# anenbergb/Co-DETR-TensorRT

Measured on AMD Instinct MI355X. Metric: images/sec, Co-DINO Swin-L 1920x1280 fp16 (p50 ms/image alongside), higher is better.
Workload: dtype f16

## Files before the change

co-detr-tensorrt_amd/csrc/gemm_xs.hip:

```cpp
#include "gemm_route.h"
#include "gemm_tile.h"

namespace {

#ifndef CODETR_XS_ABL
#define CODETR_XS_ABL 0
#endif
#ifdef CODETR_XS_STAMPS
__device__ unsigned long long* g_xs_stamps = nullptr;
#define XS_STAMP(i) xs_t[i] = __builtin_readcyclecounter()
#else
#define XS_STAMP(i)
#endif
struct XsPosGen {
  const float* ycum[5];
  const float* xcum[5];
  const unsigned short* level_embed;
  int H[5], W[5], start[5];
  int L, S;
  float log2_temperature, scale, eps, offset;
  int normalize;
};

template <class T, int KS, int ACT, bool HAS_RES, class OT = T, bool SPLIT = false, bool POSGEN = false>
__global__ __launch_bounds__(256) void linear_xs_kernel(const unsigned short* __restrict__ X,
                                                        const unsigned short* __restrict__ X2,
                                                        const unsigned short* __restrict__ LNG,
                                                        const unsigned short* __restrict__ LNB, float ln_eps,
                                                        const unsigned short* __restrict__ W,
                                                        const unsigned short* __restrict__ bias,
                                                        const unsigned short* __restrict__ R,
                                                        unsigned short* __restrict__ Y,
                                                        const unsigned char* __restrict__ row_mask, int M, int N, int hm_rows,
                                                        int hm_hd, unsigned short* __restrict__ Y2 = nullptr, int N1 = 0,
                                                        const XsPosGen pg = XsPosGen()) {
  constexpr int K = KS * 32, CH = K / 8;
  constexpr int CN = 32;
  constexpr int kChunkBytes = CN * K * 2;
  constexpr int kPieces = kChunkBytes / 4096;
  constexpr int kXsPitch = 2 * CN * 2 + 16;
  constexpr int kStage = 4 * 32 * kXsPitch;
  constexpr int kMaxBias = 1568;
  constexpr int SWZ = (CH % 16 == 0) ? 15 : 7;
  constexpr int kRing = 3;
  constexpr int kLeBytes = POSGEN ? 5 * K * 2 : 0;
  __shared__ __attribute__((aligned(16))) unsigned char lds[kRing * kChunkBytes + kStage + kMaxBias * 2 + kLeBytes];
  unsigned char* stage_base = lds + kRing * kChunkBytes;
  unsigned short* sBias = reinterpret_cast<unsigned short*>(lds + kRing * kChunkBytes + kStage);
  unsigned short* sLe = sBias + kMaxBias;
  const int tid = threadIdx.x, lane = tid & 63;
  const int wave = __builtin_amdgcn_readfirstlane(tid >> 6);
  const int l15 = lane & 15, grp = lane >> 4;
  const int m0 = (int)xcd_tile(blockIdx.x, gridDim.x) * 128 + wave * 32;
  const int nchunks = (N + CN - 1) / CN;
#ifdef CODETR_XS_STAMPS
  unsigned long long xs_t[8], xs_acc[6] = {0, 0, 0, 0, 0, 0};
  const unsigned long long xs_start = __builtin_readcyclecounter(), xs_rt0 = __builtin_amdgcn_s_memrealtime();
#endif
  const int Ny = SPLIT ? N1 : N;
  const int c1 = SPLIT ? N1 / CN : 0;

  unsigned piece_row[kPieces], piece_off[kPieces];
#pragma unroll
  for (int q = 0; q < kPieces; ++q) {
    const int u = q * 256 + tid;
    const int r = u / CH, pos = u % CH;
    piece_row[q] = (unsigned)r;
    piece_off[q] = (unsigned)((pos ^ (r & SWZ)) * 16);
  }
  const unsigned char* Wb = reinterpret_cast<const unsigned char*>(W);
  auto stage_chunk = [&](int c, unsigned char* dst) {
    const unsigned rmax = (unsigned)(N - 1 - c * CN);
#pragma unroll
    for (int q = 0; q < kPieces; ++q) {
      const unsigned r = piece_row[q] < rmax ? piece_row[q] : rmax;
      lds_dma16(Wb + (size_t)c * kChunkBytes, r * (unsigned)(K * 2) + piece_off[q], dst + (q * 256 + wave * 64) * 16);
    }
  };
  stage_chunk(0, lds);
  stage_chunk(nchunks > 1 ? 1 : 0, lds + kChunkBytes);

  typename T::frag xf[2][KS];
#pragma unroll
  for (int mt = 0; mt < 2; ++mt) {
    int m = m0 + mt * 16 + l15;
    m = m < M ? m : M - 1;
#pragma unroll
    for (int ks = 0; ks < KS; ++ks) {
      if (CODETR_XS_ABL & 16) {
#pragma unroll
        for (int e = 0; e < 8; ++e) xf[mt][ks][e] = (typename T::elem)(float)(m + ks);
        continue;
      }
      xf[mt][ks] = *reinterpret_cast<const typename T::frag*>(X + (size_t)m * K + ks * 32 + grp * 8);
    }
    if (X2 && !SPLIT && !(CODETR_XS_ABL & 16)) {
#pragma unroll
      for (int ks = 0; ks < KS; ++ks) {
        const typename T::frag p = *reinterpret_cast<const typename T::frag*>(X2 + (size_t)m * K + ks * 32 + grp * 8);
#pragma unroll
        for (int e = 0; e < 8; ++e) xf[mt][ks][e] = (typename T::elem)((float)xf[mt][ks][e] + (float)p[e]);
      }
    }
    if (LNG) {
      float sm = 0.f;
#pragma unroll
      for (int ks = 0; ks < KS; ++ks)
#pragma unroll
        for (int e = 0; e < 8; ++e) sm += (float)xf[mt][ks][e];
      sm += __shfl_xor(sm, 16, 64);
      sm += __shfl_xor(sm, 32, 64);
      const float mean = sm * (1.0f / K);
      float q = 0.f;
#pragma unroll
      for (int ks = 0; ks < KS; ++ks)
#pragma unroll
        for (int e = 0; e < 8; ++e) {
          const float d = (float)xf[mt][ks][e] - mean;
          q = fmaf(d, d, q);
        }
      q += __shfl_xor(q, 16, 64);
      q += __shfl_xor(q, 32, 64);
      const float rstd = rsqrtf(q * (1.0f / K) + ln_eps);
#pragma unroll
      for (int ks = 0; ks < KS; ++ks) {
        const typename T::frag gw = *reinterpret_cast<const typename T::frag*>(LNG + ks * 32 + grp * 8);
        const typename T::frag gb = *reinterpret_cast<const typename T::frag*>(LNB + ks * 32 + grp * 8);
#pragma unroll
        for (int e = 0; e < 8; ++e)
          xf[mt][ks][e] = (typename T::elem)fmaf(((float)xf[mt][ks][e] - mean) * rstd, (float)gw[e], (float)gb[e]);
      }
    }
  }
  float pg_ey[2] = {0.f, 0.f}, pg_ex[2] = {0.f, 0.f};
  int pg_lv[2] = {0, 0};
  if constexpr (POSGEN) {
#pragma unroll
    for (int mt = 0; mt < 2; ++mt) {
      int m = m0 + mt * 16 + l15;
      m = m < M ? m : M - 1;
      const int b = m / pg.S, tok = m - b * pg.S;
      int l = 0;
#pragma unroll
      for (int k = 1; k < 5; ++k) l += (k < pg.L && tok >= pg.start[k]) ? 1 : 0;
      int Hl = pg.H[0], Wl = pg.W[0], st = pg.start[0];
      const float* yc = pg.ycum[0];
      const float* xc = pg.xcum[0];
#pragma unroll
      for (int k = 1; k < 5; ++k) {
        const bool me = l == k;
        Hl = me ? pg.H[k] : Hl;
        Wl = me ? pg.W[k] : Wl;
        st = me ? pg.start[k] : st;
        yc = me ? pg.ycum[k] : yc;
        xc = me ? pg.xcum[k] : xc;
      }
      const int r = tok - st, y = r / Wl, x = r - y * Wl;
      const int64_t base = (int64_t)b * Hl * Wl;
      float ey = yc[base + r], ex = xc[base + r];
      if (pg.normalize) {
        const float ly = yc[base + (int64_t)(Hl - 1) * Wl + x], lx = xc[base + (int64_t)y * Wl + (Wl - 1)];
        ey = (ey + pg.offset) / (ly + pg.eps) * pg.scale;
        ex = (ex + pg.offset) / (lx + pg.eps) * pg.scale;
      }
      pg_ey[mt] = ey;
      pg_ex[mt] = ex;
      pg_lv[mt] = l;
    }
    if (pg.level_embed)
      for (int i = tid; i < pg.L * K / 8; i += 256)
        *reinterpret_cast<s16x8*>(sLe + i * 8) = *reinterpret_cast<const s16x8*>(pg.level_embed + i * 8);
  }
  if (bias) {
    for (int i = tid; i < N / 8; i += 256)
      *reinterpret_cast<s16x8*>(sBias + i * 8) = *reinterpret_cast<const s16x8*>(bias + i * 8);
  }
  unsigned row_states = 0;
  if (row_mask) {
#pragma unroll
    for (int it = 0; it < 4; ++it) {
      const int m = m0 + it * 8 + (lane >> 3);
      row_states |= (m < M ? (unsigned)row_mask[m] : 0u) << (8 * it);
    }
  }
  asm volatile("s_waitcnt lgkmcnt(0)" ::: "memory");

  unsigned char* my_stage = stage_base + wave * (32 * kXsPitch);
  const int srow = lane >> 3, schunk = lane & 7;
  s16x8 rr[4];
  auto load_residual = [&](int np) {
#pragma unroll
    for (int it = 0; it < 4; ++it) {
      int m = m0 + it * 8 + srow;
      m = m < M ? m : M - 1;
      const int n = epi_residual_col(np + schunk * 8, N);
      rr[it] = *reinterpret_cast<const s16x8*>(R + (size_t)m * N + n);
    }
  };
  auto flush_pair = [&](int np) {
    __builtin_amdgcn_wave_barrier();
#pragma unroll
    for (int it = 0; it < 4; ++it) {
      const int ml = it * 8 + srow;
      const int m = m0 + ml;
      const int n = np + schunk * 8;
      s16x8 v = *reinterpret_cast<const s16x8*>(my_stage + ml * kXsPitch + schunk * 16);
      if (SPLIT && np >= N1) {
        if (m < M && n < N) *reinterpret_cast<s16x8*>(Y2 + (size_t)m * (N - N1) + (n - N1)) = v;
        continue;
      }
      if (m < M && n < Ny) {
        if (row_mask)
          epi_row_state<T, OT, ACT, HAS_RES>(v, (unsigned char)((row_states >> (8 * it)) & 0xffu), bias != nullptr, sBias, n);
        if (HAS_RES) {
#pragma unroll
          for (int e = 0; e < 8; ++e) v[e] = (short)epi_residual<T, ACT>((unsigned short)v[e], (unsigned short)rr[it][e]);
        }
        size_t off = (size_t)m * Ny + n;
        if (hm_hd > 0) off = epi_head_major(m, n, Ny, hm_rows, hm_hd);
        if (!(CODETR_XS_ABL & 1) || v[0] == 0x1234) *reinterpret_cast<s16x8*>(Y + off) = v;
      }
    }
    __builtin_amdgcn_wave_barrier();
  };
  int slot = 0;
#ifdef CODETR_XS_STAMPS
  const unsigned long long xs_loop = __builtin_readcyclecounter();
#endif
  for (int c = 0; c < nchunks; ++c) {
    XS_STAMP(0);
    if (!(CODETR_XS_ABL & 8)) wait_vmcnt<kPieces>();
    XS_STAMP(1);
    if (!(CODETR_XS_ABL & 8)) __builtin_amdgcn_s_barrier();
    XS_STAMP(2);
    const int n0 = c * CN;
    if (!(c & 1)) {
      if (c >= 2) flush_pair((c - 2) * CN);
    } else if (HAS_RES) {
      load_residual((c - 1) * CN);
    }
    XS_STAMP(3);
    {
      const int c2 = c + 2 < nchunks ? c + 2 : nchunks - 1;
      const int s2 = slot == 0 ? 2 : slot - 1;
      if (!(CODETR_XS_ABL & 4)) stage_chunk(c2, lds + s2 * kChunkBytes);
    }
    XS_STAMP(4);
    if (SPLIT && c == c1) {
#pragma unroll
      for (int mt = 0; mt < 2; ++mt) {
        int m = m0 + mt * 16 + l15;
        m = m < M ? m : M - 1;
        if constexpr (POSGEN) {
          static_assert(!POSGEN || KS == 8, "256 channels");
          constexpr int num_feats = K / 2;
#pragma unroll
          for (int ks = 0; ks < KS; ++ks) {
            typename T::frag pfk;
            const float e_ = ks >= KS / 2 ? pg_ex[mt] : pg_ey[mt];
            const int ch0 = (4 * (ks & 3) + grp) * 8;
#pragma unroll
            for (int p = 0; p < 4; ++p) {
              const int f = (ch0 >> 1) + p;
              const float inv = __builtin_amdgcn_exp2f(-pg.log2_temperature * (2.0f * (float)f / (float)num_feats));
              const float rev = e_ * inv * 0.15915494309189535f;
              pfk[2 * p] = (typename T::elem)__builtin_amdgcn_sinf(rev);
              pfk[2 * p + 1] = (typename T::elem)__builtin_amdgcn_cosf(rev);
            }
            if (pg.level_embed) {
              const typename T::frag le = *reinterpret_cast<const typename T::frag*>(sLe + pg_lv[mt] * K + (4 * ks + grp) * 8);
#pragma unroll
              for (int k = 0; k < 8; ++k) pfk[k] = (typename T::elem)((float)pfk[k] + (float)le[k]);
            }
#pragma unroll
            for (int e = 0; e < 8; ++e) xf[mt][ks][e] = (typename T::elem)((float)xf[mt][ks][e] + (float)pfk[e]);
            asm volatile("" : "+v"(pg_ey[mt]), "+v"(pg_ex[mt]));
          }
        } else {
          typename T::frag pf[KS];
#pragma unroll
          for (int ks = 0; ks < KS; ++ks)
            pf[ks] = *reinterpret_cast<const typename T::frag*>(X2 + (size_t)m * K + ks * 32 + grp * 8);
#pragma unroll
          for (int ks = 0; ks < KS; ++ks)
#pragma unroll
            for (int e = 0; e < 8; ++e) xf[mt][ks][e] = (typename T::elem)((float)xf[mt][ks][e] + (float)pf[ks][e]);
        }
      }
    }
    const unsigned char* sW = lds + slot * kChunkBytes;
    slot = slot == 2 ? 0 : slot + 1;

    f32x4 acc[2][2];
#pragma unroll
    for (int nt = 0; nt < 2; ++nt) {
      f32x4 b4 = {0.f, 0.f, 0.f, 0.f};
      if (bias) {
        const s16x4 bv = *reinterpret_cast<const s16x4*>(sBias + n0 + nt * 16 + grp * 4);
#pragma unroll
        for (int r = 0; r < 4; ++r) b4[r] = T::to_f32((unsigned short)bv[r]);
      }
      acc[nt][0] = b4;
      acc[nt][1] = b4;
    }
#pragma unroll
    for (int ks = 0; ks < KS; ++ks) {
      typename T::frag a[2];
#pragma unroll
      for (int nt = 0; nt < 2; ++nt) {
        const int row = nt * 16 + l15;
        const int chunk = (ks * 4 + grp) ^ (row & SWZ);
        a[nt] = *reinterpret_cast<const typename T::frag*>(sW + row * (K * 2) + chunk * 16);
      }
#pragma unroll
      for (int nt = 0; nt < 2; ++nt)
#pragma unroll
        for (int mt = 0; mt < 2; ++mt) {
          if (CODETR_XS_ABL & 2) acc[nt][mt][0] += (float)a[nt][0] * (float)xf[mt][ks][0];
          else acc[nt][mt] = T::mfma(a[nt], xf[mt][ks], acc[nt][mt]);
        }
    }
#ifdef CODETR_XS_STAMPS
    asm volatile("" ::"v"(acc[1][1][3]) : "memory");
#endif
    XS_STAMP(5);
#pragma unroll
    for (int nt = 0; nt < 2; ++nt)
#pragma unroll
      for (int mt = 0; mt < 2; ++mt) {
        float v[4];
#pragma unroll
        for (int r = 0; r < 4; ++r) v[r] = epi_act<ACT, HAS_RES>(acc[nt][mt][r]);
        *reinterpret_cast<s16x4*>(my_stage + (mt * 16 + l15) * kXsPitch + ((c & 1) * CN + nt * 16 + grp * 4) * 2) =
            (SPLIT && c >= c1) ? T::pack4(v) : OT::pack4(v);
      }
#ifdef CODETR_XS_STAMPS
    asm volatile("" ::: "memory");
    XS_STAMP(6);
#pragma unroll
    for (int i = 0; i < 6; ++i) xs_acc[i] += xs_t[i + 1] - xs_t[i];
#endif
  }
  {
    const int np = ((nchunks - 1) & ~1) * CN;
    if (HAS_RES && (nchunks & 1)) load_residual(np);
    flush_pair(np);
  }
  wait_vmcnt<0>();
#ifdef CODETR_XS_STAMPS
  if (threadIdx.x == 0 && g_xs_stamps) {
    unsigned long long* o = g_xs_stamps + 12 * (size_t)blockIdx.x;
#pragma unroll
    for (int i = 0; i < 6; ++i) o[i] = xs_acc[i];
    o[6] = xs_loop - xs_start;
    o[7] = __builtin_readcyclecounter() - xs_start;
    o[8] = xs_rt0;
    o[9] = __builtin_amdgcn_s_memrealtime();
  }
#endif
}

using gemm_route::xs_applicable;

template <class T, int KS, int ACT, class OT = T>
int launch_xs_res(hipStream_t st, const void* X, const void* W, const void* bias, const void* R, void* Y,
                  const void* mask, int M, int N, int hm_rows, int hm_hd, const void* X2 = nullptr,
                  const void* LNG = nullptr, const void* LNB = nullptr, float ln_eps = 0.f) {
  const dim3 grid((unsigned)((M + 127) / 128)), block(256);
  const Operands o(X, W, bias, R, Y, mask);
  if (R && std::is_same<T, OT>::value)
    hipLaunchKernelGGL((linear_xs_kernel<T, KS, ACT, true, T>), grid, block, 0, st, o.x, u16(X2), u16(LNG), u16(LNB), ln_eps, o.w, o.b, o.r, o.y, o.mk, M, N, hm_rows, hm_hd);
  else if (R) return CODETR_E_UNSUPPORTED;
  else hipLaunchKernelGGL((linear_xs_kernel<T, KS, ACT, false, OT>), grid, block, 0, st, o.x, u16(X2), u16(LNG), u16(LNB), ln_eps, o.w, o.b, o.r, o.y, o.mk, M, N, hm_rows, hm_hd);
  const hipError_t err = hipGetLastError();
  return err == hipSuccess ? 0 : (int)err;
}

template <class T>
int launch_xadd(hipStream_t st, const void* X, const void* X2, const void* W, const void* bias, void* Y, int64_t M,
                int64_t N, int64_t K) {
  if (!X || !X2 || !W || !Y || M <= 0 || N <= 0 || K <= 0) return CODETR_E_BADARG;
  if (M > 0x7fffffffLL || N > 0x7fffffffLL) return CODETR_E_TOO_LARGE;
  if (!xs_applicable(M, N, K, 0) || K == 64 || !aligned16(Y, X, X2, W)) return CODETR_E_UNSUPPORTED;
  return dispatch_ks(K, [&](auto ks) {
    return launch_xs_res<T, ks(), 0>(st, X, W, bias, nullptr, Y, nullptr, (int)M, (int)N, 0, 0, X2);
  });
}

template <class T>
int launch_ln(hipStream_t st, const void* X, const void* G, const void* Bt, float eps, const void* W, const void* bias,
              void* Y, int64_t M, int64_t N, int64_t K, int act) {
  if (!X || !G || !Bt || !W || !Y || M <= 0 || N <= 0 || K <= 0 || act < 0 || act > 2) return CODETR_E_BADARG;
  if (M > 0x7fffffffLL || N > 0x7fffffffLL) return CODETR_E_TOO_LARGE;
  if (!xs_applicable(M, N, K, 0) || K == 64 || !aligned16(Y, X, G, Bt, W)) return CODETR_E_UNSUPPORTED;
  return dispatch_act(act, [&](auto a) {
    return dispatch_ks(K, [&](auto ks) {
      return launch_xs_res<T, ks(), a()>(st, X, W, bias, nullptr, Y, nullptr, (int)M, (int)N, 0, 0, nullptr, G, Bt, eps);
    });
  });
}

int split_check(const void* X, const void* second, const void* W, const void* bias, const void* Y, const void* Y2, int64_t M,
                int64_t N1, int64_t N2, int64_t K, int64_t hm_rows, int hm_hd, int own = 0) {
  if (!X || !W || !Y || !Y2 || M <= 0 || N1 <= 0 || N2 <= 0 || K <= 0) return CODETR_E_BADARG;
  if (own) return own;
  if (M > 0x7fffffffLL) return CODETR_E_TOO_LARGE;
  if (!aligned16(X, second, W, Y, Y2, bias)) return CODETR_E_BADARG;
  if (hm_hd != 0 || hm_rows != 0) {
    if (hm_hd <= 0 || hm_rows <= 0 || hm_hd % 8 != 0 || N1 % hm_hd != 0 || M % hm_rows != 0) return CODETR_E_UNSUPPORTED;
  }
  if (K != 256 || N1 % 64 != 0 || N2 % 8 != 0 || N1 + N2 > 1536 || M < 128 * 256) return CODETR_E_UNSUPPORTED;
  return 0;
}

template <class T, class OT>
int launch_split(hipStream_t st, const void* X, const void* X2, const void* W, const void* bias, const void* mask, void* Y,
                 void* Y2, int64_t M, int64_t N1, int64_t N2, int64_t K, int64_t hm_rows, int hm_hd) {
  if (!X2) return CODETR_E_BADARG;
  if (const int rc = split_check(X, X2, W, bias, Y, Y2, M, N1, N2, K, hm_rows, hm_hd)) return rc;
  const dim3 grid((unsigned)((M + 127) / 128)), block(256);
  const Operands o(X, W, bias, nullptr, Y, mask);
  hipLaunchKernelGGL((linear_xs_kernel<T, 8, 0, false, OT, true>), grid, block, 0, st, o.x, u16(X2), nullptr, nullptr, 0.f,
                     o.w, o.b, nullptr, o.y, o.mk, (int)M, (int)(N1 + N2), (int)hm_rows, hm_hd,
                     static_cast<unsigned short*>(Y2), (int)N1);
  const hipError_t err = hipGetLastError();
  return err == hipSuccess ? 0 : (int)err;
}

template <class T, class OT>
int launch_split_pos(hipStream_t st, const void* X, const float* const* ycum, const float* const* xcum,
                     const int64_t* shapes, int L, const void* level_embed, float temperature, float scale, float eps,
                     float offset, int normalize, const void* W, const void* bias, const void* mask, void* Y, void* Y2,
                     int64_t M, int64_t S, int64_t N1, int64_t N2, int64_t K, int64_t hm_rows, int hm_hd) {
  if (!ycum || !xcum || !shapes || S <= 0 || L <= 0 || !(temperature > 0.f)) return CODETR_E_BADARG;
  const int own = L > 5 ? CODETR_E_UNSUPPORTED : M % S != 0 ? CODETR_E_BADARG : 0;
  if (const int rc = split_check(X, level_embed, W, bias, Y, Y2, M, N1, N2, K, hm_rows, hm_hd, own)) return rc;
  XsPosGen pg;
  int64_t sum = 0;
  for (int l = 0; l < 5; ++l) {
    pg.ycum[l] = l < L ? ycum[l] : nullptr;
    pg.xcum[l] = l < L ? xcum[l] : nullptr;
    const int64_t h = l < L ? shapes[2 * l] : 1, w = l < L ? shapes[2 * l + 1] : 1;
    if (l < L && (!ycum[l] || !xcum[l] || h <= 0 || w <= 0 || h > 32767 || w > 32767)) return CODETR_E_BADARG;
    pg.H[l] = (int)h;
    pg.W[l] = (int)w;
    pg.start[l] = l < L ? (int)sum : 0x7fffffff;
    if (l < L) sum += h * w;
  }
  if (sum != S) return CODETR_E_BADARG;
  pg.level_embed = u16(level_embed);
  pg.L = L;
  pg.S = (int)S;
  pg.log2_temperature = log2f(temperature);
  pg.scale = scale;
  pg.eps = eps;
  pg.offset = offset;
  pg.normalize = normalize;
  const dim3 grid((unsigned)((M + 127) / 128)), block(256);
  const Operands o(X, W, bias, nullptr, Y, mask);
  hipLaunchKernelGGL((linear_xs_kernel<T, 8, 0, false, OT, true, true>), grid, block, 0, st, o.x, nullptr, nullptr, nullptr,
                     0.f, o.w, o.b, nullptr, o.y, o.mk, (int)M, (int)(N1 + N2), (int)hm_rows, hm_hd,
                     static_cast<unsigned short*>(Y2), (int)N1, pg);
  const hipError_t err = hipGetLastError();
  return err == hipSuccess ? 0 : (int)err;
}

}

bool gemm_route::xs_applicable(int64_t M, int64_t N, int64_t K, int hm_hd) {
  return (K == 192 || K == 256 || K == 64) && N % 8 == 0 && N >= 128 && N <= 1536 && M >= 128 * 256 && hm_hd % 8 == 0;
}

int gemm_route::launch_xs(hipStream_t st, bool bf16, const void* X, const void* W, const void* bias, const void* R, void* Y,
                          const void* mask, int M, int N, int K, int act, int hm_rows, int hm_hd) {
  return dispatch_elem(bf16, [&](auto t) {
    using T = decltype(t);
    if (K == 64) return launch_xs_res<T, 2, 0>(st, X, W, bias, nullptr, Y, mask, M, N, hm_rows, hm_hd);
    return dispatch_ks(K, [&](auto ks) {
      return dispatch_act(act, [&](auto a) { return launch_xs_res<T, ks(), a()>(st, X, W, bias, R, Y, mask, M, N, hm_rows, hm_hd); });
    });
  });
}

extern "C" {

int codetr_encoder_projections_posgen_f16(void* stream, const void* x_dev, const float* ycum0, const float* ycum1,
                                          const float* ycum2, const float* ycum3, const float* ycum4, const float* xcum0,
                                          const float* xcum1, const float* xcum2, const float* xcum3, const float* xcum4,
                                          const int64_t* level_shapes_host, int num_levels, const void* level_embed_dev,
                                          float temperature, float scale, float eps, float offset, int normalize,
                                          const void* w_dev, const void* bias_dev, const void* row_mask_dev, void* value_dev,
                                          void* packed_dev, int64_t M, int64_t S, int64_t N_value, int64_t N_packed, int64_t K,
                                          int64_t hm_rows, int hm_head_dim) {
  const float* yc[5] = {ycum0, ycum1, ycum2, ycum3, ycum4};
  const float* xc[5] = {xcum0, xcum1, xcum2, xcum3, xcum4};
  return launch_split_pos<HalfT, HalfT>(static_cast<hipStream_t>(stream), x_dev, yc, xc, level_shapes_host, num_levels,
                                        level_embed_dev, temperature, scale, eps, offset, normalize, w_dev, bias_dev, row_mask_dev,
                                        value_dev, packed_dev, M, S, N_value, N_packed, K, hm_rows, hm_head_dim);
}

int codetr_encoder_projections_posgen_bf16(void* stream, const void* x_dev, const float* ycum0, const float* ycum1,
                                          const float* ycum2, const float* ycum3, const float* ycum4, const float* xcum0,
                                          const float* xcum1, const float* xcum2, const float* xcum3, const float* xcum4,
                                          const int64_t* level_shapes_host, int num_levels, const void* level_embed_dev,
                                          float temperature, float scale, float eps, float offset, int normalize,
                                          const void* w_dev, const void* bias_dev, const void* row_mask_dev, void* value_f16_dev,
                                          void* packed_dev, int64_t M, int64_t S, int64_t N_value, int64_t N_packed, int64_t K,
                                          int64_t hm_rows, int hm_head_dim) {
  const float* yc[5] = {ycum0, ycum1, ycum2, ycum3, ycum4};
  const float* xc[5] = {xcum0, xcum1, xcum2, xcum3, xcum4};
  return launch_split_pos<BFloatT, HalfT>(static_cast<hipStream_t>(stream), x_dev, yc, xc, level_shapes_host, num_levels,
                                        level_embed_dev, temperature, scale, eps, offset, normalize, w_dev, bias_dev, row_mask_dev,
                                        value_f16_dev, packed_dev, M, S, N_value, N_packed, K, hm_rows, hm_head_dim);
}

int codetr_encoder_projections_f16(void* stream, const void* x_dev, const void* pos_dev, const void* w_dev,
                                   const void* bias_dev, const void* row_mask_dev, void* value_dev, void* packed_dev,
                                   int64_t M, int64_t N_value, int64_t N_packed, int64_t K, int64_t hm_rows, int hm_head_dim) {
  return launch_split<HalfT, HalfT>(static_cast<hipStream_t>(stream), x_dev, pos_dev, w_dev, bias_dev, row_mask_dev,
                                    value_dev, packed_dev, M, N_value, N_packed, K, hm_rows, hm_head_dim);
}

int codetr_encoder_projections_bf16(void* stream, const void* x_dev, const void* pos_dev, const void* w_dev,
                                    const void* bias_dev, const void* row_mask_dev, void* value_f16_dev, void* packed_dev,
                                    int64_t M, int64_t N_value, int64_t N_packed, int64_t K, int64_t hm_rows,
                                    int hm_head_dim) {
  return launch_split<BFloatT, HalfT>(static_cast<hipStream_t>(stream), x_dev, pos_dev, w_dev, bias_dev, row_mask_dev,
                                      value_f16_dev, packed_dev, M, N_value, N_packed, K, hm_rows, hm_head_dim);
}

int codetr_linear_ln_f16(void* stream, const void* x_dev, const void* ln_gamma_dev, const void* ln_beta_dev, float ln_eps,
                         const void* w_dev, const void* bias_dev, void* y_dev, int64_t M, int64_t N, int64_t K, int act) {
  return launch_ln<HalfT>(static_cast<hipStream_t>(stream), x_dev, ln_gamma_dev, ln_beta_dev, ln_eps, w_dev, bias_dev,
                          y_dev, M, N, K, act);
}

int codetr_linear_ln_bf16(void* stream, const void* x_dev, const void* ln_gamma_dev, const void* ln_beta_dev, float ln_eps,
                          const void* w_dev, const void* bias_dev, void* y_dev, int64_t M, int64_t N, int64_t K, int act) {
  return launch_ln<BFloatT>(static_cast<hipStream_t>(stream), x_dev, ln_gamma_dev, ln_beta_dev, ln_eps, w_dev, bias_dev,
                            y_dev, M, N, K, act);
}

int codetr_linear_xadd_f16(void* stream, const void* x_dev, const void* x_add_dev, const void* w_dev,
                           const void* bias_dev, void* y_dev, int64_t M, int64_t N, int64_t K) {
  return launch_xadd<HalfT>(static_cast<hipStream_t>(stream), x_dev, x_add_dev, w_dev, bias_dev, y_dev, M, N, K);
}

int codetr_linear_xadd_bf16(void* stream, const void* x_dev, const void* x_add_dev, const void* w_dev,
                            const void* bias_dev, void* y_dev, int64_t M, int64_t N, int64_t K) {
  return launch_xadd<BFloatT>(static_cast<hipStream_t>(stream), x_dev, x_add_dev, w_dev, bias_dev, y_dev, M, N, K);
}

int codetr_linear_bf16_f16out(void* stream, const void* x_dev, const void* w_dev, const void* bias_dev,
                              const void* row_mask_dev, void* y_dev, int64_t M, int64_t N, int64_t K, int64_t hm_rows,
                              int hm_head_dim) {
  if (!x_dev || !w_dev || !y_dev || M <= 0 || N <= 0 || K <= 0) return CODETR_E_BADARG;
  if (M > 0x7fffffffLL || N > 0x7fffffffLL) return CODETR_E_TOO_LARGE;
  if (!aligned16(x_dev, w_dev, y_dev)) return CODETR_E_BADARG;
  if (hm_head_dim != 0 || hm_rows != 0) {
    if (hm_head_dim <= 0 || hm_rows <= 0 || hm_head_dim % 8 != 0 || N % hm_head_dim != 0 || M % hm_rows != 0) return CODETR_E_UNSUPPORTED;
  }
  if (!xs_applicable(M, N, K, hm_head_dim) || K == 64) return CODETR_E_UNSUPPORTED;
  hipStream_t st = static_cast<hipStream_t>(stream);
  return dispatch_ks(K, [&](auto ks) {
    return launch_xs_res<BFloatT, ks(), 0, HalfT>(st, x_dev, w_dev, bias_dev, nullptr, y_dev, row_mask_dev, (int)M, (int)N,
                                                  (int)hm_rows, hm_head_dim);
  });
}

}
```

Baseline: 99.44.

## Interleave epilogue flush, residual loads and weight staging into the MFMA k-loop

For KS>2, the chunk body is software-pipelined. LDS weight fragments are read kAhead steps early, and the previous pair's flush rows, residual row loads and per-piece DMA staging of the next-next chunk are spread across the MFMA k-steps, separated by sched_barriers. The loop is unrolled by two with a compile-time odd/even tag so parity branches fold away. The aim is to hide epilogue store and global load latency behind matrix math instead of serializing them before the k-loop. In exchange the code is more complex, register pressure rises from the extra fragment buffers, and the sched_barriers pin a fixed instruction order.

Measured after the change: 99.93 (median of 6 runs). No clear change (+0.5%).

```diff
diff --git a/co-detr-tensorrt_amd/csrc/gemm_xs.hip b/co-detr-tensorrt_amd/csrc/gemm_xs.hip
--- a/co-detr-tensorrt_amd/csrc/gemm_xs.hip
+++ b/co-detr-tensorrt_amd/csrc/gemm_xs.hip
@@ -69,13 +69,14 @@
     piece_off[q] = (unsigned)((pos ^ (r & SWZ)) * 16);
   }
   const unsigned char* Wb = reinterpret_cast<const unsigned char*>(W);
-  auto stage_chunk = [&](int c, unsigned char* dst) {
+  auto stage_piece = [&](int c, unsigned char* dst, int q) __attribute__((always_inline)) {
     const unsigned rmax = (unsigned)(N - 1 - c * CN);
-#pragma unroll
-    for (int q = 0; q < kPieces; ++q) {
-      const unsigned r = piece_row[q] < rmax ? piece_row[q] : rmax;
-      lds_dma16(Wb + (size_t)c * kChunkBytes, r * (unsigned)(K * 2) + piece_off[q], dst + (q * 256 + wave * 64) * 16);
-    }
+    const unsigned r = piece_row[q] < rmax ? piece_row[q] : rmax;
+    lds_dma16(Wb + (size_t)c * kChunkBytes, r * (unsigned)(K * 2) + piece_off[q], dst + (q * 256 + wave * 64) * 16);
+  };
+  auto stage_chunk = [&](int c, unsigned char* dst) __attribute__((always_inline)) {
+#pragma unroll
+    for (int q = 0; q < kPieces; ++q) stage_piece(c, dst, q);
   };
   stage_chunk(0, lds);
   stage_chunk(nchunks > 1 ? 1 : 0, lds + kChunkBytes);
@@ -188,64 +189,80 @@
   unsigned char* my_stage = stage_base + wave * (32 * kXsPitch);
   const int srow = lane >> 3, schunk = lane & 7;
   s16x8 rr[4];
-  auto load_residual = [&](int np) {
-#pragma unroll
-    for (int it = 0; it < 4; ++it) {
-      int m = m0 + it * 8 + srow;
-      m = m < M ? m : M - 1;
-      const int n = epi_residual_col(np + schunk * 8, N);
-      rr[it] = *reinterpret_cast<const s16x8*>(R + (size_t)m * N + n);
-    }
-  };
-  auto flush_pair = [&](int np) {
+  auto load_residual_row = [&](int np, int it) __attribute__((always_inline)) {
+    int m = m0 + it * 8 + srow;
+    m = m < M ? m : M - 1;
+    const int n = epi_residual_col(np + schunk * 8, N);
+    rr[it] = *reinterpret_cast<const s16x8*>(R + (size_t)m * N + n);
+  };
+  auto load_residual = [&](int np) __attribute__((always_inline)) {
+#pragma unroll
+    for (int it = 0; it < 4; ++it) load_residual_row(np, it);
+  };
+  auto flush_read = [&](int it) __attribute__((always_inline)) {
+    return *reinterpret_cast<const s16x8*>(my_stage + (it * 8 + srow) * kXsPitch + schunk * 16);
+  };
+  auto flush_row = [&](int np, int it, s16x8 v, bool live) __attribute__((always_inline)) {
+    const int m = m0 + it * 8 + srow;
+    const int n = np + schunk * 8;
+    if (SPLIT && np >= N1) {
+      if (live && m < M && n < N) *reinterpret_cast<s16x8*>(Y2 + (size_t)m * (N - N1) + (n - N1)) = v;
+      return;
+    }
+    if (live && m < M && n < Ny) {
+      if (row_mask)
+        epi_row_state<T, OT, ACT, HAS_RES>(v, (unsigned char)((row_states >> (8 * it)) & 0xffu), bias != nullptr, sBias, n);
+      if (HAS_RES) {
+#pragma unroll
+        for (int e = 0; e < 8; ++e) v[e] = (short)epi_residual<T, ACT>((unsigned short)v[e], (unsigned short)rr[it][e]);
+      }
+      size_t off = (size_t)m * Ny + n;
+      if (hm_hd > 0) off = epi_head_major(m, n, Ny, hm_rows, hm_hd);
+      if (!(CODETR_XS_ABL & 1) || v[0] == 0x1234) *reinterpret_cast<s16x8*>(Y + off) = v;
+    }
+  };
+  auto flush_pair = [&](int np) __attribute__((always_inline)) {
     __builtin_amdgcn_wave_barrier();
 #pragma unroll
-    for (int it = 0; it < 4; ++it) {
-      const int ml = it * 8 + srow;
-      const int m = m0 + ml;
-      const int n = np + schunk * 8;
-      s16x8 v = *reinterpret_cast<const s16x8*>(my_stage + ml * kXsPitch + schunk * 16);
-      if (SPLIT && np >= N1) {
-        if (m < M && n < N) *reinterpret_cast<s16x8*>(Y2 + (size_t)m * (N - N1) + (n - N1)) = v;
-        continue;
-      }
-      if (m < M && n < Ny) {
-        if (row_mask)
-          epi_row_state<T, OT, ACT, HAS_RES>(v, (unsigned char)((row_states >> (8 * it)) & 0xffu), bias != nullptr, sBias, n);
-        if (HAS_RES) {
-#pragma unroll
-          for (int e = 0; e < 8; ++e) v[e] = (short)epi_residual<T, ACT>((unsigned short)v[e], (unsigned short)rr[it][e]);
-        }
-        size_t off = (size_t)m * Ny + n;
-        if (hm_hd > 0) off = epi_head_major(m, n, Ny, hm_rows, hm_hd);
-        if (!(CODETR_XS_ABL & 1) || v[0] == 0x1234) *reinterpret_cast<s16x8*>(Y + off) = v;
-      }
-    }
+    for (int it = 0; it < 4; ++it) flush_row(np, it, flush_read(it), true);
     __builtin_amdgcn_wave_barrier();
+  };
+  constexpr bool kPipelined = KS != 2;
+  constexpr int kAhead = KS > 2 ? 2 : 1;
+  constexpr int kFlushSlots = KS - kPieces;
+  static_assert(kFlushSlots >= 1 && kAhead >= 1 && kAhead < KS, "slot plan");
+  auto read_w = [&](const unsigned char* sW, int ks, typename T::frag(&a)[2]) __attribute__((always_inline)) {
+#pragma unroll
+    for (int nt = 0; nt < 2; ++nt) {
+      const int row = nt * 16 + l15;
+      const int chunk = (ks * 4 + grp) ^ (row & SWZ);
+      a[nt] = *reinterpret_cast<const typename T::frag*>(sW + row * (K * 2) + chunk * 16);
+    }
   };
   int slot = 0;
 #ifdef CODETR_XS_STAMPS
   const unsigned long long xs_loop = __builtin_readcyclecounter();
 #endif
-  for (int c = 0; c < nchunks; ++c) {
+  auto chunk_body = [&](auto odd_tag, const int c) __attribute__((always_inline)) {
+    const bool ODD = odd_tag;
     XS_STAMP(0);
     if (!(CODETR_XS_ABL & 8)) wait_vmcnt<kPieces>();
     XS_STAMP(1);
     if (!(CODETR_XS_ABL & 8)) __builtin_amdgcn_s_barrier();
     XS_STAMP(2);
     const int n0 = c * CN;
-    if (!(c & 1)) {
-      if (c >= 2) flush_pair((c - 2) * CN);
-    } else if (HAS_RES) {
-      load_residual((c - 1) * CN);
-    }
-    XS_STAMP(3);
-    {
-      const int c2 = c + 2 < nchunks ? c + 2 : nchunks - 1;
-      const int s2 = slot == 0 ? 2 : slot - 1;
-      if (!(CODETR_XS_ABL & 4)) stage_chunk(c2, lds + s2 * kChunkBytes);
-    }
-    XS_STAMP(4);
+    const int c2 = c + 2 < nchunks ? c + 2 : nchunks - 1;
+    unsigned char* const dW2 = lds + (slot == 0 ? 2 : slot - 1) * kChunkBytes;
+    if constexpr (!kPipelined) {
+      if (!ODD) {
+        if (c >= 2) flush_pair((c - 2) * CN);
+      } else if (HAS_RES) {
+        load_residual((c - 1) * CN);
+      }
+      XS_STAMP(3);
+      if (!(CODETR_XS_ABL & 4)) stage_chunk(c2, dW2);
+      XS_STAMP(4);
+    }
     if (SPLIT && c == c1) {
 #pragma unroll
       for (int mt = 0; mt < 2; ++mt) {
@@ -292,26 +309,21 @@
     slot = slot == 2 ? 0 : slot + 1;
 
     f32x4 acc[2][2];
-#pragma unroll
-    for (int nt = 0; nt < 2; ++nt) {
-      f32x4 b4 = {0.f, 0.f, 0.f, 0.f};
-      if (bias) {
-        const s16x4 bv = *reinterpret_cast<const s16x4*>(sBias + n0 + nt * 16 + grp * 4);
-#pragma unroll
-        for (int r = 0; r < 4; ++r) b4[r] = T::to_f32((unsigned short)bv[r]);
-      }
-      acc[nt][0] = b4;
-      acc[nt][1] = b4;
-    }
-#pragma unroll
-    for (int ks = 0; ks < KS; ++ks) {
-      typename T::frag a[2];
+    s16x4 bv[2];
+#pragma unroll
+    for (int nt = 0; nt < 2; ++nt) bv[nt] = *reinterpret_cast<const s16x4*>(sBias + n0 + nt * 16 + grp * 4);
+    auto init_acc = [&]() __attribute__((always_inline)) {
 #pragma unroll
       for (int nt = 0; nt < 2; ++nt) {
-        const int row = nt * 16 + l15;
-        const int chunk = (ks * 4 + grp) ^ (row & SWZ);
-        a[nt] = *reinterpret_cast<const typename T::frag*>(sW + row * (K * 2) + chunk * 16);
-      }
+        f32x4 b4;
+#pragma unroll
+        for (int r = 0; r < 4; ++r) b4[r] = bias ? T::to_f32((unsigned short)bv[nt][r]) : 0.f;
+        acc[nt][0] = b4;
+        acc[nt][1] = b4;
+      }
+    };
+    if constexpr (!kPipelined) init_acc();
+    auto mfma_step = [&](int ks, const typename T::frag(&a)[2]) __attribute__((always_inline)) {
 #pragma unroll
       for (int nt = 0; nt < 2; ++nt)
 #pragma unroll
@@ -319,6 +331,52 @@
           if (CODETR_XS_ABL & 2) acc[nt][mt][0] += (float)a[nt][0] * (float)xf[mt][ks][0];
           else acc[nt][mt] = T::mfma(a[nt], xf[mt][ks], acc[nt][mt]);
         }
+    };
+    if constexpr (kPipelined) {
+      typename T::frag a[kAhead + 1][2];
+#pragma unroll
+      for (int ks = 0; ks < kAhead; ++ks) read_w(sW, ks, a[ks]);
+      init_acc();
+      const int np = (c - (ODD ? 1 : 2)) * CN;
+      if (!ODD) __builtin_amdgcn_wave_barrier();
+      XS_STAMP(3);
+#pragma unroll
+      for (int ks = 0; ks < KS; ++ks) {
+#ifdef CODETR_XS_STAMPS
+        if (ks == kFlushSlots) {
+          XS_STAMP(4);
+        }
+#endif
+        s16x8 fv[4];
+        if (!ODD) {
+#pragma unroll
+          for (int it = 0; it < 4; ++it)
+            if (it * kFlushSlots / 4 == ks) fv[it] = flush_read(it);
+        }
+        if (ks + kAhead < KS) read_w(sW, ks + kAhead, a[(ks + kAhead) % (kAhead + 1)]);
+        __builtin_amdgcn_sched_barrier(0);
+        mfma_step(ks, a[ks % (kAhead + 1)]);
+        __builtin_amdgcn_sched_barrier(0);
+#pragma unroll
+        for (int it = 0; it < 4; ++it)
+          if (it * kFlushSlots / 4 == ks) {
+            if (!ODD) {
+              flush_row(np, it, fv[it], c >= 2);
+              if (it == 3) __builtin_amdgcn_wave_barrier();
+            } else if (HAS_RES) {
+              load_residual_row(np, it);
+            }
+          }
+        if (ks >= kFlushSlots && !(CODETR_XS_ABL & 4)) stage_piece(c2, dW2, ks - kFlushSlots);
+        __builtin_amdgcn_sched_barrier(0);
+      }
+    } else {
+#pragma unroll
+      for (int ks = 0; ks < KS; ++ks) {
+        typename T::frag a[2];
+        read_w(sW, ks, a);
+        mfma_step(ks, a);
+      }
     }
 #ifdef CODETR_XS_STAMPS
     asm volatile("" ::"v"(acc[1][1][3]) : "memory");
@@ -331,7 +389,7 @@
         float v[4];
 #pragma unroll
         for (int r = 0; r < 4; ++r) v[r] = epi_act<ACT, HAS_RES>(acc[nt][mt][r]);
-        *reinterpret_cast<s16x4*>(my_stage + (mt * 16 + l15) * kXsPitch + ((c & 1) * CN + nt * 16 + grp * 4) * 2) =
+        *reinterpret_cast<s16x4*>(my_stage + (mt * 16 + l15) * kXsPitch + ((ODD ? CN : 0) + nt * 16 + grp * 4) * 2) =
             (SPLIT && c >= c1) ? T::pack4(v) : OT::pack4(v);
       }
 #ifdef CODETR_XS_STAMPS
@@ -340,6 +398,14 @@
 #pragma unroll
     for (int i = 0; i < 6; ++i) xs_acc[i] += xs_t[i + 1] - xs_t[i];
 #endif
+  };
+  if constexpr (kPipelined) {
+    for (int c = 0; c < nchunks; c += 2) {
+      chunk_body(std::false_type(), c);
+      if (c + 1 < nchunks) chunk_body(std::true_type(), c + 1);
+    }
+  } else {
+    for (int c = 0; c < nchunks; ++c) chunk_body((c & 1) != 0, c);
   }
   {
     const int np = ((nchunks - 1) & ~1) * CN;
```
